# wenet-e2e/wetts

Hardware: AMD Instinct MI355X
Metric: audio samples/sec + RTF @22.05 kHz, VITS-Baker, 1/2/4/8 MI355X (higher is better)
Workload: dtype f32

## Files before the change

wetts_amd/csrc/kernels.h:

```cpp
#pragma once
#include "common.h"

namespace wetts {

int32_t k_embed_mask(const int64_t* ids, const int64_t* lengths, const float* emb, int n_vocab,
                     int B, int H, int T, float* x_out, float* mask_out, int32_t* status,
                     hipStream_t s);

int32_t k_layernorm(const float* a, const float* add, const float* gamma, const float* beta,
                    const float* res, const float* mask, int gelu, int B, int C, int T, float* out,
                    hipStream_t s);

struct DdsFusedParams {
  const float* x;
  float* out;
  const float* mask;
  const float *sep_w[3], *sep_b[3], *n1g[3], *n1b[3], *n2g[3], *n2b[3];
  const float* wpk[3];
  const float* bias[3];
  int B, C, T, G;
};
bool dds_fused_supported(int mode, int C, int Cw, int nchunks, int B, int T);
int32_t k_dds_fused(DdsFusedParams p, hipStream_t s);
int32_t k_dwconv(const float* x, const float* mask, const float* w, const float* bias, int k,
                 int dil, int B, int C, int T, float* out, hipStream_t s, int Tvalid = 0);

int32_t k_cond_linear(const float* g, const float* W, const float* bias, int B, int Cout, int K,
                      float* out, hipStream_t s);

int32_t k_gather_rows(const int64_t* idx, const float* table, int n_rows, int B, int C, float* out,
                      int32_t* status, hipStream_t s);

int32_t k_add_bias_b(float* x, const float* v, int B, int C, int T, hipStream_t s);
int32_t k_add_bias_b_mask(float* x, const float* v, const float* mask, int B, int C, int T,
                          hipStream_t s);
int32_t k_scale(const float* a, float scale, int64_t n, float* out, hipStream_t s);

int32_t k_convflow_pre(const float* z, int ch0, const float* w, const float* bias, const float* g,
                       int B, int C, int T, float* out, hipStream_t s);

int32_t k_spline_inverse(float* z, int ch0, int ch1, const float* h, const float* mask,
                         int num_bins, float tail_bound, float inv_sqrt_div, int B, int T,
                         int32_t* status, hipStream_t s);

int32_t k_affine_reverse(const float* z, int ch, const float* m, const float* logs, int param_idx,
                         const float* mask, int B, int T, float* logw, hipStream_t s);

int32_t k_gate(const float* a, int B, int H, int T, float* out, hipStream_t s);

int32_t k_wn_update(const float* rs, float* h, float* skip, const float* mask, int last, int first,
                    int B, int H, int T, hipStream_t s);

int32_t k_coupling_flip(const float* xin, const float* m, const float* mask, int B, int C, int T,
                        float* out, hipStream_t s);

int32_t k_conv_post_tanh(const float* x, const float* w, int k, int B, int C, int T, float* out,
                         hipStream_t s, const int64_t* lens = nullptr, int len_mul = 0);

int32_t k_durations_to_lengths(const float* logw, const float* mask, float length_scale, int B,
                               int T, float* w_ceil, float* cum, int64_t* y_lengths,
                               int32_t* status, hipStream_t s);

int32_t k_frame_index(const float* cum, const int64_t* y_lengths, int B, int Tx, int Ty,
                      int32_t* frame2phone, float* y_mask, hipStream_t s);
int32_t k_expand_prior(const float* stats, const int32_t* frame2phone, const float* eps,
                       int64_t eps_bs, int64_t eps_cs, float noise_scale, int B, int C, int Tx, int Ty, float* m_exp,
                       float* logs_exp, float* z_p, hipStream_t s);
int32_t k_attn_path(const int32_t* frame2phone, int B, int Tx, int Ty, float* attn, hipStream_t s);

int32_t k_audio_to_int16(const float* audio, const int64_t* lengths, int B, int64_t L, int16_t* pcm,
                         hipStream_t s);

int32_t k_vocos_pad(const float* z, int64_t z_bs, int64_t z_cs, const float* mask,
                    int64_t mask_stride, int B, int C, int L, float* out, hipStream_t s, int Fs = 0);
int32_t k_vocos_spec(const float* spec, int B, int half, int F, float* ri, hipStream_t s, int64_t ri_bs = 0);
int32_t k_istft_basis(int n_fft, float* w, hipStream_t s, double inv_scale = 0.0);
bool k_convnext_dwln(const float* x, const float* w, const float* wb, const float* gamma, const float* beta, int B, int C,
                     int T, int Tvalid, float* out, hipStream_t s, int32_t* rc);
int32_t k_istft_ola(const float* frames, int B, int n_fft, int hop, int F, float* audio,
                    hipStream_t s, int Fs = 0, int envelope = 1);
int32_t k_scale_rows(const float* a, const float* scale, int rows, int cols, float* out,
                     hipStream_t s);

int32_t k_flip_half(const float* x, const float* mask, int B, int C, int T, float* x0, float* x0m,
                    hipStream_t s);
int32_t k_mono_split(const float* x, const float* mask, int B, int C, int T, float sc, float* x0, float* x0m,
                     hipStream_t s);
int32_t k_mono_coupling(const float* x, const float* m, const float* mask, int B, int C, int T, float sc, float* out,
                        hipStream_t s);
int32_t k_coupling_fwd_flip(const float* x, const float* m, const float* mask, int B, int C, int T, float* out,
// ... 35 lines not shown
```

wetts_amd/csrc/kernels.hip:

```cpp
#include "kernels.h"

namespace wetts {

static inline dim3 grid1d(int64_t n, int threads) {
  return dim3((unsigned)((n + threads - 1) / threads));
}

__global__ void embed_mask_kernel(const int64_t* __restrict__ ids,
                                  const int64_t* __restrict__ lengths,
                                  const float* __restrict__ emb, int n_vocab, int B, int H, int T,
                                  float scale, float* __restrict__ x_out,
                                  float* __restrict__ mask_out, int32_t* __restrict__ status) {
  int64_t idx = (int64_t)blockIdx.x * blockDim.x + threadIdx.x;
  int64_t total = (int64_t)B * H * T;
  if (idx >= total) return;
  int t = (int)(idx % T);
  int c = (int)((idx / T) % H);
  int b = (int)(idx / ((int64_t)T * H));
  bool valid = (int64_t)t < lengths[b];
  float v = 0.f;
  if (valid) {
    int64_t id = ids[(int64_t)b * T + t];
    if (id < 0 || id >= n_vocab) {
      if (status && c == 0) atomicOr(status, WETTS_STATUS_PHONE_ID_RANGE);
// ... 663 lines not shown
  const float* xb = x + (int64_t)b * C * T;
  float win[MAXC][K], wv[MAXC][K];
#pragma unroll
  for (int j = 0; j < MAXC; ++j) {
    const int c = cg + CG * j;
    const int cc = c < C ? c : 0;
#pragma unroll
    for (int i = 0; i < K; ++i) {
      const int tt = t - pad + i;
      const bool ok = c < C && tt >= 0 && tt < T;
      win[j][i] = xb[(int64_t)cc * T + (ok ? tt : 0)];
      wv[j][i] = ok ? w[cc * K + i] : 0.f;
    }
  }
  float acc = 0.f;
#pragma unroll
  for (int j = 0; j < MAXC; ++j)
#pragma unroll
    for (int i = 0; i < K; ++i) {
      const float v = win[j][i];
      acc += wv[j][i] * (v > 0.f ? v : v * 0.01f);
    }
  red[cg][tl] = acc;
  __syncthreads();
  if (cg == 0 && t < T) {
    float tot = 0.f;
#pragma unroll
    for (int q = 0; q < CG; ++q) tot += red[q][tl];
    out[(int64_t)b * T + t] = tanhf(tot);
  }
}

int32_t k_conv_post_tanh(const float* x, const float* w, int k, int B, int C, int T, float* out,
                         hipStream_t s, const int64_t* lens, int len_mul) {
  WETTS_REQUIRE(k <= 15, "conv_post kernel size %d unsupported", k);
  int64_t n = (int64_t)B * ((T + 3) / 4);
  if (n == 0) return WETTS_OK;
  if (k == 7 && C <= 64 && n <= 64 * 256 && !lens) {
    hipLaunchKernelGGL(conv_post_tanh_small_kernel<7>, dim3((unsigned)(B * cdiv(T, 32))), dim3(256), 0, s, x, w,
                       B, C, T, out);
    WETTS_LAUNCH_CHECK();
    return WETTS_OK;
  }
  hipLaunchKernelGGL(conv_post_tanh_kernel, grid1d(n, 256), dim3(256), (size_t)C * k * 4, s, x, w,
                     k, B, C, T, out, lens, len_mul);
  WETTS_LAUNCH_CHECK();
  return WETTS_OK;
}

__global__ __launch_bounds__(64) void durations_kernel(const float* __restrict__ logw,
                                                       const float* __restrict__ mask,
                                                       float length_scale, int B, int T,
                                                       float* __restrict__ w_ceil,
                                                       float* __restrict__ cum,
                                                       int64_t* __restrict__ y_lengths,
                                                       int32_t* __restrict__ status) {
  const int b = blockIdx.x, lane = threadIdx.x;
  float carry = 0.f;
  for (int t0 = 0; t0 < T; t0 += 64) {
    int t = t0 + lane;
    float wc = 0.f;
    if (t < T) {
      float w = expf(logw[(int64_t)b * T + t]) * mask[(int64_t)b * T + t] * length_scale;
      wc = ceilf(w);
      w_ceil[(int64_t)b * T + t] = wc;
    }
    float v = wc;
#pragma unroll
    for (int off = 1; off < 64; off <<= 1) {
      float n = __shfl_up(v, off, 64);
      if (lane >= off) v += n;
// ... 548 lines not shown
```

wetts_amd/csrc/model.hip:

```cpp
#include <stdarg.h>
#include <stdlib.h>
#include <string.h>

#include <map>
#include <string>
#include <vector>

#include "common.h"
#include "conv_bf16.h"
#include "resblock32.h"
#include "qconv_u8.h"
#include "kernels.h"

namespace wetts {

static thread_local char g_err[512] = "";

void set_error(const char* fmt, ...) {
  va_list ap;
  va_start(ap, fmt);
  vsnprintf(g_err, sizeof(g_err), fmt, ap);
  va_end(ap);
}

// ... 394 lines not shown
  int fuse32_maxc = 32;
  int fuse32_kmax = 99;
  int fuse32_kwide = 3;
  int fuse2_maxc = 128;
  int fuse_min_blocks = 128;
  int small_max_tiles = 256;
  int chain_whole_waste_pct = 15;
  int chain_whole_maxc = 64;
  int chain_pair_maxc = 32;
  int chain_pair_kmax = 3;
  int fuse2_waste_pct = 20;
  mutable int flow_precision = 0;
  mutable std::vector<std::vector<PackedConvB>> b_wn_in, b_wn_rs;
  mutable PackedConvB b_post;
  mutable float* b_post_wpad = nullptr;
  mutable PackedQConv q_pre, q_cond, q_post;
  mutable std::vector<std::vector<PackedQConv>> q_c1, q_c2;
  mutable bool q_packed = false;
  mutable int flow_packed_prec = 0, dec_packed_prec = 0;
  mutable std::vector<PackedConvB> b_ups;
  mutable PackedConvB b_pre;
  mutable std::vector<std::vector<PackedConvB>> b_c1, b_c2;
  mutable int32_t* status_word = nullptr;
  mutable uint64_t rng_seed = 0, rng_offset = 0;
  int mrf_streams = 1;
  int mrf_fork_maxc = 1 << 20;
  int stage2_pct = 30;
  int dds_fused = 1;
  int wn_gate = 1;
  int wn_fuse = 1;
  int small_fork = 1;
  int conv_groups = 1;
  hipStream_t aux_stream[WETTS_MAX_RB_KERNELS] = {};
  hipEvent_t ev_fork = nullptr, ev_chain[WETTS_MAX_RB_KERNELS] = {};
  bool fork_ok = false;

  int spec_channels = 0;
  bool post_loaded = false;
  Layout post_layout;
  float* post_blob = nullptr;
  PackedConv pe_pre, pe_proj;
  std::vector<PackedConv> pe_in, pe_rs, fwd_pre;
  const float *pe_cond_w = nullptr, *pe_cond_b = nullptr;

  const float* T(const std::string& name) const {
    auto it = layout.index.find(name);
    if (it == layout.index.end()) return nullptr;
    return blob + layout.specs[it->second].offset;
  }
};

namespace wetts {

struct Bump {
  char* base;
  int64_t cap, off = 0;
  bool ok = true;
  Bump(void* p, int64_t c) : base((char*)p), cap(c) {}
  template <typename T>
  T* take(int64_t n) {
    int64_t bytes = align_up(n * (int64_t)sizeof(T), 256);
    if (off + bytes > cap) {
      ok = false;
      return nullptr;
    }
    T* r = (T*)(base + off);
    off += bytes;
    return r;
// ... 426 lines not shown
  return L.total;
}

int32_t wetts_create(const wetts_config_t* cfg, const float* blob_dev, int64_t blob_numel,
                     void* stream, wetts_model_t** out) {
  WETTS_TRY(validate_config(cfg));
  WETTS_REQUIRE(out != nullptr && blob_dev != nullptr, "null argument");
  hipStream_t s = (hipStream_t)stream;
  wetts_model* m = new wetts_model();
  m->cfg = *cfg;
  build_layout(cfg, m->layout);
  if (blob_numel != m->layout.total) {
    set_error("blob has %lld floats, layout needs %lld", (long long)blob_numel,
              (long long)m->layout.total);
    delete m;
    return WETTS_E_INVALID;
  }
  hipError_t e = hipMalloc((void**)&m->blob, (size_t)blob_numel * sizeof(float));
  if (e != hipSuccess) {
    set_error("hipMalloc(blob) failed: %s", hipGetErrorString(e));
    delete m;
    return WETTS_E_HIP;
  }
  e = hipMemcpyAsync(m->blob, blob_dev, (size_t)blob_numel * sizeof(float),
                     hipMemcpyDeviceToDevice, s);
  int32_t r = (e == hipSuccess) ? build_model(m, s) : WETTS_E_HIP;
  {
    struct Knob { const char* name; int* field; };
    const Knob knobs[] = {
        {"stage2_pct", &m->stage2_pct}, {"dds_fused", &m->dds_fused}, {"wn_fuse", &m->wn_fuse}, {"wn_gate", &m->wn_gate},
        {"fuse2_waste_pct", &m->fuse2_waste_pct}, {"fuse_min_blocks", &m->fuse_min_blocks},
        {"chain_whole_pct", &m->chain_whole_waste_pct}, {"chain_whole_maxc", &m->chain_whole_maxc},
        {"small_max_tiles", &m->small_max_tiles},
    };
    if (const char* env = getenv("WETTS_TUNE")) {
      std::string all(env);
      size_t pos = 0;
      while (pos < all.size()) {
        size_t end = all.find(',', pos);
        if (end == std::string::npos) end = all.size();
        const std::string item = all.substr(pos, end - pos);
        const size_t eq = item.find('=');
        bool known = false;
        if (eq != std::string::npos)
          for (const Knob& k : knobs)
            if (item.compare(0, eq, k.name) == 0 && strlen(k.name) == eq) {
              *k.field = atoi(item.c_str() + eq + 1);
              known = true;
            }
        if (!known && !item.empty()) {
          set_error("WETTS_TUNE: unknown setting '%s'", item.c_str());
          r = WETTS_E_INVALID;
        }
        pos = end + 1;
      }
    }
    if (r == WETTS_OK && !m->wn_gate) {
      const int H = cfg->hidden_channels, fk = cfg->flow_kernel_size;
      for (int f = 0; f < cfg->flow_n_flows && r == WETTS_OK; ++f)
        for (int i = 0; i < cfg->flow_wn_layers && r == WETTS_OK; ++i) {
          const std::string p = S("flow.flows.%d.enc.in_layers.%d", flow_key_stride(cfg) * f, i);
          free_packed(&m->flows[f].in_layers[i]);
          r = pack_conv_weight(m->T(p + ".weight"), m->T(p + ".bias"), 2 * H, H, fk, 1, (fk - 1) / 2, 0, 0, s,
                               &m->flows[f].in_layers[i]);
        }
    }
    if (m->mrf_streams < 1) m->mrf_streams = 1;
    if (m->mrf_streams > cfg->n_resblock_kernels) m->mrf_streams = cfg->n_resblock_kernels;
    m->fork_ok = hipEventCreateWithFlags(&m->ev_fork, hipEventDisableTiming) == hipSuccess && m->ev_fork;
    for (int j = 0; j < cfg->n_resblock_kernels; ++j) {
      if (hipEventCreateWithFlags(&m->ev_chain[j], hipEventDisableTiming) != hipSuccess || !m->ev_chain[j]) m->fork_ok = false;
      if (j > 0)
        if (hipStreamCreateWithFlags(&m->aux_stream[j], hipStreamNonBlocking) != hipSuccess || !m->aux_stream[j]) m->fork_ok = false;
    }
    (void)hipGetLastError();
  }
  if (r == WETTS_OK) {
    e = hipStreamSynchronize(s);
    if (e != hipSuccess) {
      set_error("weight packing failed: %s", hipGetErrorString(e));
      r = WETTS_E_HIP;
    }
  }
  if (r != WETTS_OK) {
    wetts_destroy(m);
    return r;
  }
  *out = m;
  return WETTS_OK;
}

void wetts_destroy(wetts_model_t* m) {
  if (!m) return;
  free_posterior(m);
  for (PackedConv* pc : m->all_packed) free_packed(pc);
  for (auto& pc : m->b_ups) free_packed_bf16(&pc);
  for (auto& v : m->b_c1) for (auto& pc : v) free_packed_bf16(&pc);
  for (auto& v : m->b_c2) for (auto& pc : v) free_packed_bf16(&pc);
  for (auto& v : m->b_wn_in) for (auto& pc : v) free_packed_bf16(&pc);
  for (auto& v : m->b_wn_rs) for (auto& pc : v) free_packed_bf16(&pc);
  free_packed_bf16(&m->b_post);
  if (m->b_post_wpad) (void)hipFree(m->b_post_wpad);
  free_packed_qconv(&m->q_pre);
  free_packed_qconv(&m->q_cond);
  free_packed_qconv(&m->q_post);
  for (auto& v : m->q_c1) for (auto& pc : v) free_packed_qconv(&pc);
  for (auto& v : m->q_c2) for (auto& pc : v) free_packed_qconv(&pc);
  for (int j = 0; j < WETTS_MAX_RB_KERNELS; ++j) {
    if (m->aux_stream[j]) (void)hipStreamDestroy(m->aux_stream[j]);
    if (m->ev_chain[j]) (void)hipEventDestroy(m->ev_chain[j]);
  }
  if (m->ev_fork) (void)hipEventDestroy(m->ev_fork);
  for (float* p : m->v_owned) (void)hipFree(p);
  if (m->blob) (void)hipFree(m->blob);
  delete m;
}

int32_t wetts_hop_length(const wetts_model_t* m) { return m ? m->hop : WETTS_E_INVALID; }

int32_t wetts_set_istft_mode(const wetts_model_t* m, int32_t mode) {
  WETTS_REQUIRE(m, "null model");
  WETTS_REQUIRE(mode == WETTS_ISTFT_TORCH || mode == WETTS_ISTFT_ONNX, "istft mode must be 0 (torch.istft) or 1 (OnnxSTFT.inverse), got %d", mode);
  m->istft_mode = mode;
  return WETTS_OK;
}

int32_t wetts_get_istft_mode(const wetts_model_t* m) { return m ? m->istft_mode : WETTS_E_INVALID; }

int32_t wetts_get_blob(const wetts_model_t* m, float* out_dev, int64_t numel, void* stream) {
  WETTS_REQUIRE(m && out_dev, "null argument");
  WETTS_REQUIRE(numel == m->layout.total, "blob has %lld floats, asked for %lld", (long long)m->layout.total,
                (long long)numel);
  WETTS_HIP_CHECK(hipMemcpyAsync(out_dev, m->blob, (size_t)numel * sizeof(float), hipMemcpyDeviceToDevice,
                                 (hipStream_t)stream));
  return WETTS_OK;
}

int64_t wetts_workspace_bytes(const wetts_model_t* m, int32_t B, int32_t Tx, int32_t Ty) {
  if (!m || B < 0 || Tx < 0 || Ty < 0) return WETTS_E_INVALID;
  const wetts_config_t* c = &m->cfg;
  int64_t a = ws_encoder(c, B, Tx);
  int64_t b = c->use_sdp ? ws_sdp(c, B, Tx) : ws_dp(c, B, Tx);
  int64_t need = a > b ? a : b;
  if (Ty > 0) {
    int64_t f = ws_flow(c, B, Ty), d = ws_decoder(c, B, Ty);
// ... 1001 lines not shown
        WETTS_TRY(launch_resblock_pair32(rb.c1[d], rb.c2[d], pp, s));
        count(1, 2 + accum);
      } else {
        ConvParams p2 = conv_io(chain_buf[j][2], ch, len, outp[j], ch, B);
        p2.in_act = IN_LRELU;
        p2.in_slope = 0.1f;
        p2.res = rx[j];
        p2.r_bs = (int64_t)ch * len;
        p2.r_cs = len;
        p2.accum = accum;
        p2.out_div = odiv;
        p2.tag = 1;
        p2.lens = lens;
        p2.len_mul = spf;
        if (last_d || m->dec_unfused) {
          WETTS_TRY(launch_conv(rb.c2[d], p2, s));
          count(1, 3 + accum);
        } else {
          g2[n2] = &rb.c2[d];
          p2s[n2++] = p2;
        }
      }
      rx[j] = outp[j];
    }
    if (n2 > 0) {
      int nl = 0;
      WETTS_TRY(launch_conv_group(g2, p2s, n2, s, &nl));
      count(nl, 3.0 * n2);
    }
  }
  return WETTS_OK;
}

static int32_t run_hifigan(const wetts_model* m, const float* z, int64_t z_bs, int64_t z_cs,
                           const float* y_mask, int64_t mask_stride, const float* g, int B, int L,
                           float* audio, void* workspace, int64_t workspace_bytes, hipStream_t s,
                           DecTiming* tm, const int64_t* lens = nullptr) {
  const wetts_config_t* c = &m->cfg;
  const int I = c->inter_channels, C0 = c->upsample_initial_channel;
  const int64_t mx = dec_max_elems(c, B, L);
  Bump ws(workspace, workspace_bytes);
  float* bx = ws.take<float>(mx);
  float* bt = ws.take<float>(mx);
  float* bs = ws.take<float>(mx);
  float* chain_buf[WETTS_MAX_RB_KERNELS][3];
  for (int j = 0; j < c->n_resblock_kernels; ++j)
    for (int q = 0; q < 3; ++q) chain_buf[j][q] = ws.take<float>(mx);
  float* cond = ws.take<float>((int64_t)B * C0);
  if (!ws.ok) {
    set_error("hifigan: workspace too small (need %lld bytes)",
              (long long)ws_decoder(c, B, L));
    return WETTS_E_WORKSPACE;
  }
  {
    ConvParams p = conv_io(z, I, L, bx, C0, B);
    p.x_bs = z_bs;
    p.x_cs = z_cs;
    if (y_mask) {
      p.in_mask = y_mask;
      p.in_mask_stride = mask_stride;
    }
    if (has_g(c) && g) {
      WETTS_TRY(k_cond_linear(g, m->dec_cond_w, m->dec_cond_b, B, C0, c->gin_channels, cond, s));
      p.bias_b = cond;
      p.bias_b_stride = C0;
    }
    p.lens = lens;
    p.len_mul = 1;
    WETTS_TRY(launch_conv(m->conv_pre, p, s));
  }
  int ch = C0, len = L;
  int spf = 1;
  float* x = bx;
  float* xs = bs;
  const int nk = c->n_resblock_kernels, nd = c->n_resblock_dilations;
  for (int i = 0; i < c->n_upsamples; ++i) {
    const int u = c->upsample_rates[i];
    {
      ConvParams p = conv_io(x, ch, len, bt, ch / 2, B);
      p.in_act = IN_LRELU;
      p.in_slope = 0.1f;
      p.Tout = len * u;
      p.o_bs = (int64_t)(ch / 2) * len * u;
      p.o_cs = (int64_t)len * u;
      p.lens = lens;
      p.len_mul = spf;
      WETTS_TRY(launch_conv(m->ups[i], p, s));
    }
    ch /= 2;
    len *= u;
    spf *= u;
    float* xu = bt;
    float* xsum = (x == bx) ? bs : bx;
    (void)xs;
    if (tm && tm->on) WETTS_HIP_CHECK(hipEventRecord(tm->e0, s));
    hipEvent_t lv0 = nullptr, lv1 = nullptr;
    if (m->mrf_timing) {
      WETTS_HIP_CHECK(hipEventCreate(&lv0));
      WETTS_HIP_CHECK(hipEventCreate(&lv1));
      WETTS_HIP_CHECK(hipEventRecord(lv0, s));
    }
    const bool small_stage = !lens && (int64_t)cdiv(ch, 64) * cdiv(len, 64) * B <= m->small_max_tiles;
    const int nstreams = !m->fork_ok ? 1 : (c->resblock == 1 && ((m->small_fork && small_stage) || (ch <= m->mrf_fork_maxc && !m->dec_serial))) ? nk : m->mrf_streams;
    const bool forked = nstreams > 1;
    if (forked) WETTS_HIP_CHECK(hipEventRecord(m->ev_fork, s));
    const bool chain_addr_ok = (int64_t)ch * len * 4 < (int64_t)INT32_MAX;
    const bool grouped = c->resblock == 1 && !forked && m->conv_groups;
    if (grouped) WETTS_TRY(run_stage_rb1_grouped(m, i, xu, xsum, chain_buf, ch, len, spf, B, lens, tm, s));
    for (int j = 0; j < (grouped ? 0 : nk); ++j) {
      const RB& rb = m->rbs[i * nk + j];
      hipStream_t sj = (forked && j > 0 && j < nstreams) ? m->aux_stream[j] : s;
      if (sj != s) WETTS_HIP_CHECK(hipStreamWaitEvent(sj, m->ev_fork, 0));
      float* fa = chain_buf[j][0];
      float* fb = chain_buf[j][1];
      float* ft = chain_buf[j][2];
      const float* rx = xu;
      if (c->resblock == 1 && !m->dec_unfused && nd <= RESCHAIN32_MAX_PAIRS &&
          ch <= m->chain_whole_maxc && m->chain_whole_waste_pct > 0 && len % 4 == 0 && chain_addr_ok &&
          resblock_chain32_supported(rb.c1.data(), rb.c2.data(), nd, m->fuse32_lds / 2,
                                     m->chain_whole_waste_pct)) {
        int dl[RESCHAIN32_MAX_PAIRS];
        for (int d = 0; d < nd; ++d) dl[d] = rb.c1[d].dil;
        if (cdiv(len, resblock_chain32_nto(ch, rb.c1[0].ktaps, dl, nd)) * B >= m->fuse_min_blocks) {
          ResChain32Params cp;
          memset(&cp, 0, sizeof(cp));
          cp.x = rx;
          cp.out = xsum;
          cp.T = len;
          cp.B = B;
          cp.accum = (j > 0) ? 1 : 0;
          cp.out_div = (j == nk - 1) ? (float)nk : 1.f;
          cp.slope = 0.1f;
          cp.lens = lens;
          cp.len_mul = spf;
          if (forked && j > 0) WETTS_HIP_CHECK(hipStreamWaitEvent(sj, m->ev_chain[j - 1], 0));
          WETTS_TRY(launch_resblock_chain32(rb.c1.data(), rb.c2.data(), nd, cp, sj));
          if (forked) WETTS_HIP_CHECK(hipEventRecord(m->ev_chain[j], sj));
          if (tm && tm->on) tm->launches += 1;
          mrf_count(m, 1, 2 + (j > 0 ? 1 : 0), ch, len, B, 4);
          continue;
        }
      }
      for (int d = 0; d < nd; ++d) {
        const bool last_d = (d == nd - 1);
        float* outp;
        int accum = 0;
        float odiv = 1.f;
        if (last_d) {
          outp = xsum;
          accum = (j > 0) ? 1 : 0;
          odiv = (j == nk - 1) ? (float)nk : 1.f;
        } else {
          outp = (rx == fa) ? fb : fa;
        }
        if (c->resblock == 2 && nd == 2 && d == 0 && !m->dec_unfused && !forked &&
            ch <= m->fuse2_maxc &&
            resblock2_chain32_supported(rb.c1[0], rb.c1[1], m->fuse32_lds,
                                        ch <= 32 ? m->fuse2_waste_pct : (m->fuse2_waste_pct + 1) / 2) &&
            cdiv(len, pair_nto(ch, 1) - (rb.c1[1].ktaps - 1) * rb.c1[1].dil) * B >= m->fuse_min_blocks) {
          ResPair32Params pp;
          memset(&pp, 0, sizeof(pp));
          pp.x = rx;
          pp.out = xsum;
          pp.T = len;
          pp.B = B;
          pp.accum = (j > 0) ? 1 : 0;
          pp.out_div = (j == nk - 1) ? (float)nk : 1.f;
          pp.slope = 0.1f;
          WETTS_TRY(launch_resblock2_chain32(rb.c1[0], rb.c1[1], pp, sj));
          if (tm && tm->on) tm->launches += 1;
          mrf_count(m, 1, 2 + (j > 0 ? 1 : 0), ch, len, B, 4);
          rx = xsum;
          break;
        }
        const int pair_tiles = cdiv(len, pair_nto(ch, rb.c1[d].ktaps)) * B;
        const bool chain1 = c->resblock == 1 && !m->dec_unfused && len % 4 == 0 && chain_addr_ok &&
                            (ch <= m->chain_pair_maxc || rb.c1[d].ktaps <= m->chain_pair_kmax) &&
                            resblock_chain32_supported(&rb.c1[d], &rb.c2[d], 1, m->fuse32_lds / 2, 100) &&
                            pair_tiles >= m->fuse_min_blocks;
        if (chain1) {
          if (forked && last_d && j > 0) WETTS_HIP_CHECK(hipStreamWaitEvent(sj, m->ev_chain[j - 1], 0));
          ResChain32Params cp;
          memset(&cp, 0, sizeof(cp));
          cp.x = rx;
          cp.out = outp;
          cp.T = len;
          cp.B = B;
          cp.accum = accum;
          cp.out_div = odiv;
          cp.slope = 0.1f;
          cp.lens = lens;
          cp.len_mul = spf;
          WETTS_TRY(launch_resblock_chain32(&rb.c1[d], &rb.c2[d], 1, cp, sj));
          if (tm && tm->on) tm->launches += 1;
          mrf_count(m, 1, 2 + accum, ch, len, B, 4);
          rx = outp;
          continue;
        }
        const bool fuse32 = c->resblock == 1 && !m->dec_unfused && !lens &&
                            resblock_pair32_supported(rb.c1[d], rb.c2[d], m->fuse32_lds) &&
                            !(ch >= 128 && rb.c1[d].ktaps >= m->fuse32_kmax128) &&
                            (ch <= m->fuse32_maxc || rb.c1[d].ktaps <= m->fuse32_kwide) &&
                            rb.c1[d].ktaps <= m->fuse32_kmax &&
                            pair_tiles >= m->fuse_min_blocks;
        if (fuse32) {
          if (forked && last_d && j > 0) WETTS_HIP_CHECK(hipStreamWaitEvent(sj, m->ev_chain[j - 1], 0));
          ResPair32Params pp;
          memset(&pp, 0, sizeof(pp));
          pp.x = rx;
          pp.out = outp;
          pp.T = len;
          pp.B = B;
          pp.accum = accum;
          pp.out_div = odiv;
          pp.slope = 0.1f;
          WETTS_TRY(launch_resblock_pair32(rb.c1[d], rb.c2[d], pp, sj));
          if (tm && tm->on) tm->launches += 1;
          mrf_count(m, 1, 2 + accum, ch, len, B, 4);
        } else if (c->resblock == 1) {
          ConvParams p1 = conv_io(rx, ch, len, ft, ch, B);
          p1.in_act = IN_LRELU;
          p1.in_slope = 0.1f;
          p1.tag = 1;
          p1.lens = lens;
          p1.len_mul = spf;
          WETTS_TRY(launch_conv(rb.c1[d], p1, sj));
          if (forked && last_d && j > 0) WETTS_HIP_CHECK(hipStreamWaitEvent(sj, m->ev_chain[j - 1], 0));
          ConvParams p2 = conv_io(ft, ch, len, outp, ch, B);
          p2.in_act = IN_LRELU;
          p2.in_slope = 0.1f;
          p2.res = rx;
          p2.r_bs = (int64_t)ch * len;
          p2.r_cs = len;
          p2.accum = accum;
          p2.out_div = odiv;
          p2.tag = 1;
          p2.lens = lens;
          p2.len_mul = spf;
          WETTS_TRY(launch_conv(rb.c2[d], p2, sj));
          if (tm && tm->on) tm->launches += 2;
          mrf_count(m, 2, 5 + accum, ch, len, B, 4);
        } else {
          if (forked && last_d && j > 0) WETTS_HIP_CHECK(hipStreamWaitEvent(sj, m->ev_chain[j - 1], 0));
          ConvParams p1 = conv_io(rx, ch, len, outp, ch, B);
          p1.in_act = IN_LRELU;
          p1.in_slope = 0.1f;
          p1.res = rx;
          p1.r_bs = (int64_t)ch * len;
          p1.r_cs = len;
          p1.accum = accum;
          p1.out_div = odiv;
          p1.tag = 1;
          WETTS_TRY(launch_conv(rb.c1[d], p1, sj));
          if (tm && tm->on) tm->launches += 1;
          mrf_count(m, 1, 2 + accum, ch, len, B, 4);
        }
        rx = outp;
      }
      if (forked) WETTS_HIP_CHECK(hipEventRecord(m->ev_chain[j], sj));
    }
    if (forked) WETTS_HIP_CHECK(hipStreamWaitEvent(s, m->ev_chain[nk - 1], 0));
    if (m->mrf_timing) {
      WETTS_HIP_CHECK(hipEventRecord(lv1, s));
      m->mrf_events.emplace_back(lv0, lv1);
    }
    if (tm && tm->on) {
      WETTS_HIP_CHECK(hipEventRecord(tm->e1, s));
      WETTS_HIP_CHECK(hipEventSynchronize(tm->e1));
      float ms = 0.f;
      WETTS_HIP_CHECK(hipEventElapsedTime(&ms, tm->e0, tm->e1));
      tm->mrf_ms += ms;
    }
    x = xsum;
  }
  WETTS_TRY(k_conv_post_tanh(x, m->conv_post_w, 7, B, ch, len, audio, s, lens, spf));
  if (m->mrf_timing) m->mrf_calls += 1;
  return WETTS_OK;
}
}

namespace wetts {
static void free_decoder_bf16(const wetts_model* m) {
  for (auto& pc : m->b_ups) free_packed_bf16(&pc);
  for (auto& v : m->b_c1) for (auto& pc : v) free_packed_bf16(&pc);
  for (auto& v : m->b_c2) for (auto& pc : v) free_packed_bf16(&pc);
  free_packed_bf16(&m->b_post);
  free_packed_bf16(&m->b_pre);
  m->b_ups.clear();
  m->b_c1.clear();
  m->b_c2.clear();
  m->dec_packed_prec = 0;
}

static int32_t pack_decoder_bf16_layers(const wetts_model* m, int f16, hipStream_t s) {
  const wetts_config_t* c = &m->cfg;
  const int nk = c->n_resblock_kernels, nd = c->n_resblock_dilations;
  m->b_ups.resize(c->n_upsamples);
  m->b_c1.assign(c->n_upsamples * nk, std::vector<PackedConvB>(nd));
  m->b_c2.assign(c->n_upsamples * nk, std::vector<PackedConvB>(c->resblock == 1 ? nd : 0));
  int ch = c->upsample_initial_channel;
  WETTS_TRY(pack_conv_weight_bf16(m->T("dec.conv_pre.weight"), m->T("dec.conv_pre.bias"), ch, c->inter_channels, 7, 1, 3,
                                  0, 0, f16, s, &m->b_pre));
  for (int i = 0; i < c->n_upsamples; ++i) {
    const int u = c->upsample_rates[i], uk = c->upsample_kernel_sizes[i];
    WETTS_TRY(pack_conv_weight_bf16(m->T(S("dec.ups.%d.weight", i)), m->T(S("dec.ups.%d.bias", i)),
                                    ch / 2, ch, uk, 1, (uk - u) / 2, 1, u, f16, s, &m->b_ups[i]));
    ch /= 2;
    for (int j = 0; j < nk; ++j) {
// ... 784 lines not shown
```

Before: 52.71 million.

## Split HiFi-GAN decoder batch into two slices run concurrently on separate streams

Refactors the decoder into per-slice stage helpers (conv_pre, upsample, resblock chains, join, conv_post) and adds a path that splits the batch into two halves whose stages are issued interleaved with separate fork/chain events. Each half can then overlap the other's kernels on separate streams, filling the GPU when a single batch's kernels leave it underused. It is gated by a tunable dec_split and skipped when the per-half stages would be too small. The cost is extra event and stream synchronisation, smaller kernels per launch, and more complex buffer handling per slice.

```diff
diff --git a/wetts_amd/csrc/kernels.h b/wetts_amd/csrc/kernels.h
--- a/wetts_amd/csrc/kernels.h
+++ b/wetts_amd/csrc/kernels.h
@@ -55,7 +55,7 @@
                         float* out, hipStream_t s);
 
 int32_t k_conv_post_tanh(const float* x, const float* w, int k, int B, int C, int T, float* out,
-                         hipStream_t s, const int64_t* lens = nullptr, int len_mul = 0);
+                         hipStream_t s, const int64_t* lens = nullptr, int len_mul = 0, int sel_rows = 0);
 
 int32_t k_durations_to_lengths(const float* logw, const float* mask, float length_scale, int B,
                                int T, float* w_ceil, float* cum, int64_t* y_lengths,
diff --git a/wetts_amd/csrc/kernels.hip b/wetts_amd/csrc/kernels.hip
--- a/wetts_amd/csrc/kernels.hip
+++ b/wetts_amd/csrc/kernels.hip
@@ -719,11 +719,12 @@
 }
 
 int32_t k_conv_post_tanh(const float* x, const float* w, int k, int B, int C, int T, float* out,
-                         hipStream_t s, const int64_t* lens, int len_mul) {
+                         hipStream_t s, const int64_t* lens, int len_mul, int sel_rows) {
   WETTS_REQUIRE(k <= 15, "conv_post kernel size %d unsupported", k);
   int64_t n = (int64_t)B * ((T + 3) / 4);
   if (n == 0) return WETTS_OK;
-  if (k == 7 && C <= 64 && n <= 64 * 256 && !lens) {
+  const int64_t n_sel = (int64_t)(sel_rows > 0 ? sel_rows : B) * ((T + 3) / 4);
+  if (k == 7 && C <= 64 && n_sel <= 64 * 256 && !lens) {
     hipLaunchKernelGGL(conv_post_tanh_small_kernel<7>, dim3((unsigned)(B * cdiv(T, 32))), dim3(256), 0, s, x, w,
                        B, C, T, out);
     WETTS_LAUNCH_CHECK();
diff --git a/wetts_amd/csrc/model.hip b/wetts_amd/csrc/model.hip
--- a/wetts_amd/csrc/model.hip
+++ b/wetts_amd/csrc/model.hip
@@ -450,8 +450,10 @@
   int small_fork = 1;
   int conv_groups = 1;
   hipStream_t aux_stream[WETTS_MAX_RB_KERNELS] = {};
-  hipEvent_t ev_fork = nullptr, ev_chain[WETTS_MAX_RB_KERNELS] = {};
+  hipEvent_t ev_fork[2] = {}, ev_chain[2][WETTS_MAX_RB_KERNELS] = {};
   bool fork_ok = false;
+  int dec_split = 1;
+  int dec_split_min_rows = 2;
 
   int spec_channels = 0;
   bool post_loaded = false;
@@ -944,6 +946,7 @@
         {"fuse2_waste_pct", &m->fuse2_waste_pct}, {"fuse_min_blocks", &m->fuse_min_blocks},
         {"chain_whole_pct", &m->chain_whole_waste_pct}, {"chain_whole_maxc", &m->chain_whole_maxc},
         {"small_max_tiles", &m->small_max_tiles},
+        {"dec_split", &m->dec_split}, {"dec_split_min_rows", &m->dec_split_min_rows},
     };
     if (const char* env = getenv("WETTS_TUNE")) {
       std::string all(env);
@@ -979,9 +982,13 @@
     }
     if (m->mrf_streams < 1) m->mrf_streams = 1;
     if (m->mrf_streams > cfg->n_resblock_kernels) m->mrf_streams = cfg->n_resblock_kernels;
-    m->fork_ok = hipEventCreateWithFlags(&m->ev_fork, hipEventDisableTiming) == hipSuccess && m->ev_fork;
+    m->fork_ok = true;
+    for (int h = 0; h < 2; ++h) {
+      if (hipEventCreateWithFlags(&m->ev_fork[h], hipEventDisableTiming) != hipSuccess || !m->ev_fork[h]) m->fork_ok = false;
+      for (int j = 0; j < cfg->n_resblock_kernels; ++j)
+        if (hipEventCreateWithFlags(&m->ev_chain[h][j], hipEventDisableTiming) != hipSuccess || !m->ev_chain[h][j]) m->fork_ok = false;
+    }
     for (int j = 0; j < cfg->n_resblock_kernels; ++j) {
-      if (hipEventCreateWithFlags(&m->ev_chain[j], hipEventDisableTiming) != hipSuccess || !m->ev_chain[j]) m->fork_ok = false;
       if (j > 0)
         if (hipStreamCreateWithFlags(&m->aux_stream[j], hipStreamNonBlocking) != hipSuccess || !m->aux_stream[j]) m->fork_ok = false;
     }
@@ -1020,9 +1027,11 @@
   for (auto& v : m->q_c2) for (auto& pc : v) free_packed_qconv(&pc);
   for (int j = 0; j < WETTS_MAX_RB_KERNELS; ++j) {
     if (m->aux_stream[j]) (void)hipStreamDestroy(m->aux_stream[j]);
-    if (m->ev_chain[j]) (void)hipEventDestroy(m->ev_chain[j]);
-  }
-  if (m->ev_fork) (void)hipEventDestroy(m->ev_fork);
+    for (int h = 0; h < 2; ++h)
+      if (m->ev_chain[h][j]) (void)hipEventDestroy(m->ev_chain[h][j]);
+  }
+  for (int h = 0; h < 2; ++h)
+    if (m->ev_fork[h]) (void)hipEventDestroy(m->ev_fork[h]);
   for (float* p : m->v_owned) (void)hipFree(p);
   if (m->blob) (void)hipFree(m->blob);
   delete m;
@@ -2090,19 +2099,283 @@
   return WETTS_OK;
 }
 
+struct DecSlice {
+  int B = 0;
+  int Bsel = 0;
+  const float* z = nullptr;
+  const float* y_mask = nullptr;
+  const float* cond = nullptr;
+  const int64_t* lens = nullptr;
+  float* audio = nullptr;
+  float *bx = nullptr, *bt = nullptr, *bs = nullptr;
+  float* chain_buf[WETTS_MAX_RB_KERNELS][3] = {};
+  hipEvent_t ev_fork = nullptr;
+  const hipEvent_t* ev_chain = nullptr;
+  int ch = 0, len = 0, spf = 1;
+  float* x = nullptr;
+  float* xsum = nullptr;
+  bool forked = false;
+};
+
+static int32_t dec_conv_pre(const wetts_model* m, DecSlice& sl, int64_t z_bs, int64_t z_cs, int64_t mask_stride, int L,
+                            hipStream_t s) {
+  const wetts_config_t* c = &m->cfg;
+  const int C0 = c->upsample_initial_channel;
+  ConvParams p = conv_io(sl.z, c->inter_channels, L, sl.bx, C0, sl.B);
+  p.x_bs = z_bs;
+  p.x_cs = z_cs;
+  if (sl.y_mask) {
+    p.in_mask = sl.y_mask;
+    p.in_mask_stride = mask_stride;
+  }
+  if (sl.cond) {
+    p.bias_b = sl.cond;
+    p.bias_b_stride = C0;
+  }
+  p.lens = sl.lens;
+  p.len_mul = 1;
+  WETTS_TRY(launch_conv(m->conv_pre, p, s));
+  sl.ch = C0;
+  sl.len = L;
+  sl.spf = 1;
+  sl.x = sl.bx;
+  return WETTS_OK;
+}
+
+static int32_t dec_upsample(const wetts_model* m, DecSlice& sl, int i, hipStream_t s) {
+  const int u = m->cfg.upsample_rates[i];
+  const int ch = sl.ch, len = sl.len;
+  ConvParams p = conv_io(sl.x, ch, len, sl.bt, ch / 2, sl.B);
+  p.in_act = IN_LRELU;
+  p.in_slope = 0.1f;
+  p.Tout = len * u;
+  p.o_bs = (int64_t)(ch / 2) * len * u;
+  p.o_cs = (int64_t)len * u;
+  p.lens = sl.lens;
+  p.len_mul = sl.spf;
+  WETTS_TRY(launch_conv(m->ups[i], p, s));
+  sl.ch = ch / 2;
+  sl.len = len * u;
+  sl.spf *= u;
+  return WETTS_OK;
+}
+
+static int32_t dec_stage_chains(const wetts_model* m, DecSlice& sl, int i, DecTiming* tm, hipStream_t s) {
+  const wetts_config_t* c = &m->cfg;
+  const int nk = c->n_resblock_kernels, nd = c->n_resblock_dilations;
+  const int ch = sl.ch, len = sl.len, spf = sl.spf, B = sl.B, Bsel = sl.Bsel;
+  const int64_t* lens = sl.lens;
+  float* xu = sl.bt;
+  float* xsum = (sl.x == sl.bx) ? sl.bs : sl.bx;
+  sl.xsum = xsum;
+  const bool small_stage = !lens && (int64_t)cdiv(ch, 64) * cdiv(len, 64) * Bsel <= m->small_max_tiles;
+  const int nstreams = !m->fork_ok ? 1 : (c->resblock == 1 && ((m->small_fork && small_stage) || (ch <= m->mrf_fork_maxc && !m->dec_serial))) ? nk : m->mrf_streams;
+  const bool forked = nstreams > 1;
+  sl.forked = forked;
+  if (forked) WETTS_HIP_CHECK(hipEventRecord(sl.ev_fork, s));
+  const bool chain_addr_ok = (int64_t)ch * len * 4 < (int64_t)INT32_MAX;
+  const bool grouped = c->resblock == 1 && !forked && m->conv_groups;
+  if (grouped) WETTS_TRY(run_stage_rb1_grouped(m, i, xu, xsum, sl.chain_buf, ch, len, spf, B, lens, tm, s));
+  for (int j = 0; j < (grouped ? 0 : nk); ++j) {
+    const RB& rb = m->rbs[i * nk + j];
+    hipStream_t sj = (forked && j > 0 && j < nstreams) ? m->aux_stream[j] : s;
+    if (sj != s) WETTS_HIP_CHECK(hipStreamWaitEvent(sj, sl.ev_fork, 0));
+    float* fa = sl.chain_buf[j][0];
+    float* fb = sl.chain_buf[j][1];
+    float* ft = sl.chain_buf[j][2];
+    const float* rx = xu;
+    if (c->resblock == 1 && !m->dec_unfused && nd <= RESCHAIN32_MAX_PAIRS &&
+        ch <= m->chain_whole_maxc && m->chain_whole_waste_pct > 0 && len % 4 == 0 && chain_addr_ok &&
+        resblock_chain32_supported(rb.c1.data(), rb.c2.data(), nd, m->fuse32_lds / 2,
+                                   m->chain_whole_waste_pct)) {
+      int dl[RESCHAIN32_MAX_PAIRS];
+      for (int d = 0; d < nd; ++d) dl[d] = rb.c1[d].dil;
+      if (cdiv(len, resblock_chain32_nto(ch, rb.c1[0].ktaps, dl, nd)) * Bsel >= m->fuse_min_blocks) {
+        ResChain32Params cp;
+        memset(&cp, 0, sizeof(cp));
+        cp.x = rx;
+        cp.out = xsum;
+        cp.T = len;
+        cp.B = B;
+        cp.accum = (j > 0) ? 1 : 0;
+        cp.out_div = (j == nk - 1) ? (float)nk : 1.f;
+        cp.slope = 0.1f;
+        cp.lens = lens;
+        cp.len_mul = spf;
+        if (forked && j > 0) WETTS_HIP_CHECK(hipStreamWaitEvent(sj, sl.ev_chain[j - 1], 0));
+        WETTS_TRY(launch_resblock_chain32(rb.c1.data(), rb.c2.data(), nd, cp, sj));
+        if (forked) WETTS_HIP_CHECK(hipEventRecord(sl.ev_chain[j], sj));
+        if (tm && tm->on) tm->launches += 1;
+        mrf_count(m, 1, 2 + (j > 0 ? 1 : 0), ch, len, B, 4);
+        continue;
+      }
+    }
+    for (int d = 0; d < nd; ++d) {
+      const bool last_d = (d == nd - 1);
+      float* outp;
+      int accum = 0;
+      float odiv = 1.f;
+      if (last_d) {
+        outp = xsum;
+        accum = (j > 0) ? 1 : 0;
+        odiv = (j == nk - 1) ? (float)nk : 1.f;
+      } else {
+        outp = (rx == fa) ? fb : fa;
+      }
+      if (c->resblock == 2 && nd == 2 && d == 0 && !m->dec_unfused && !forked &&
+          ch <= m->fuse2_maxc &&
+          resblock2_chain32_supported(rb.c1[0], rb.c1[1], m->fuse32_lds,
+                                      ch <= 32 ? m->fuse2_waste_pct : (m->fuse2_waste_pct + 1) / 2) &&
+          cdiv(len, pair_nto(ch, 1) - (rb.c1[1].ktaps - 1) * rb.c1[1].dil) * Bsel >= m->fuse_min_blocks) {
+        ResPair32Params pp;
+        memset(&pp, 0, sizeof(pp));
+        pp.x = rx;
+        pp.out = xsum;
+        pp.T = len;
+        pp.B = B;
+        pp.accum = (j > 0) ? 1 : 0;
+        pp.out_div = (j == nk - 1) ? (float)nk : 1.f;
+        pp.slope = 0.1f;
+        WETTS_TRY(launch_resblock2_chain32(rb.c1[0], rb.c1[1], pp, sj));
+        if (tm && tm->on) tm->launches += 1;
+        mrf_count(m, 1, 2 + (j > 0 ? 1 : 0), ch, len, B, 4);
+        rx = xsum;
+        break;
+      }
+      const int pair_tiles = cdiv(len, pair_nto(ch, rb.c1[d].ktaps)) * Bsel;
+      const bool chain1 = c->resblock == 1 && !m->dec_unfused && len % 4 == 0 && chain_addr_ok &&
+                          (ch <= m->chain_pair_maxc || rb.c1[d].ktaps <= m->chain_pair_kmax) &&
+                          resblock_chain32_supported(&rb.c1[d], &rb.c2[d], 1, m->fuse32_lds / 2, 100) &&
+                          pair_tiles >= m->fuse_min_blocks;
+      if (chain1) {
+        if (forked && last_d && j > 0) WETTS_HIP_CHECK(hipStreamWaitEvent(sj, sl.ev_chain[j - 1], 0));
+        ResChain32Params cp;
+        memset(&cp, 0, sizeof(cp));
+        cp.x = rx;
+        cp.out = outp;
+        cp.T = len;
+        cp.B = B;
+        cp.accum = accum;
+        cp.out_div = odiv;
+        cp.slope = 0.1f;
+        cp.lens = lens;
+        cp.len_mul = spf;
+        WETTS_TRY(launch_resblock_chain32(&rb.c1[d], &rb.c2[d], 1, cp, sj));
+        if (tm && tm->on) tm->launches += 1;
+        mrf_count(m, 1, 2 + accum, ch, len, B, 4);
+        rx = outp;
+        continue;
+      }
+      const bool fuse32 = c->resblock == 1 && !m->dec_unfused && !lens &&
+                          resblock_pair32_supported(rb.c1[d], rb.c2[d], m->fuse32_lds) &&
+                          !(ch >= 128 && rb.c1[d].ktaps >= m->fuse32_kmax128) &&
+                          (ch <= m->fuse32_maxc || rb.c1[d].ktaps <= m->fuse32_kwide) &&
+                          rb.c1[d].ktaps <= m->fuse32_kmax &&
+                          pair_tiles >= m->fuse_min_blocks;
+      if (fuse32) {
+        if (forked && last_d && j > 0) WETTS_HIP_CHECK(hipStreamWaitEvent(sj, sl.ev_chain[j - 1], 0));
+        ResPair32Params pp;
+        memset(&pp, 0, sizeof(pp));
+        pp.x = rx;
+        pp.out = outp;
+        pp.T = len;
+        pp.B = B;
+        pp.accum = accum;
+        pp.out_div = odiv;
+        pp.slope = 0.1f;
+        WETTS_TRY(launch_resblock_pair32(rb.c1[d], rb.c2[d], pp, sj));
+        if (tm && tm->on) tm->launches += 1;
+        mrf_count(m, 1, 2 + accum, ch, len, B, 4);
+      } else if (c->resblock == 1) {
+        ConvParams p1 = conv_io(rx, ch, len, ft, ch, B);
+        p1.in_act = IN_LRELU;
+        p1.in_slope = 0.1f;
+        p1.tag = 1;
+        p1.lens = lens;
+        p1.len_mul = spf;
+        WETTS_TRY(launch_conv(rb.c1[d], p1, sj));
+        if (forked && last_d && j > 0) WETTS_HIP_CHECK(hipStreamWaitEvent(sj, sl.ev_chain[j - 1], 0));
+        ConvParams p2 = conv_io(ft, ch, len, outp, ch, B);
+        p2.in_act = IN_LRELU;
+        p2.in_slope = 0.1f;
+        p2.res = rx;
+        p2.r_bs = (int64_t)ch * len;
+        p2.r_cs = len;
+        p2.accum = accum;
+        p2.out_div = odiv;
+        p2.tag = 1;
+        p2.lens = lens;
+        p2.len_mul = spf;
+        WETTS_TRY(launch_conv(rb.c2[d], p2, sj));
+        if (tm && tm->on) tm->launches += 2;
+        mrf_count(m, 2, 5 + accum, ch, len, B, 4);
+      } else {
+        if (forked && last_d && j > 0) WETTS_HIP_CHECK(hipStreamWaitEvent(sj, sl.ev_chain[j - 1], 0));
+        ConvParams p1 = conv_io(rx, ch, len, outp, ch, B);
+        p1.in_act = IN_LRELU;
+        p1.in_slope = 0.1f;
+        p1.res = rx;
+        p1.r_bs = (int64_t)ch * len;
+        p1.r_cs = len;
+        p1.accum = accum;
+        p1.out_div = odiv;
+        p1.tag = 1;
+        WETTS_TRY(launch_conv(rb.c1[d], p1, sj));
+        if (tm && tm->on) tm->launches += 1;
+        mrf_count(m, 1, 2 + accum, ch, len, B, 4);
+      }
+      rx = outp;
+    }
+    if (forked) WETTS_HIP_CHECK(hipEventRecord(sl.ev_chain[j], sj));
+  }
+  return WETTS_OK;
+}
+
+static int32_t dec_stage_join(const wetts_model* m, DecSlice& sl, hipStream_t s) {
+  if (sl.forked) WETTS_HIP_CHECK(hipStreamWaitEvent(s, sl.ev_chain[m->cfg.n_resblock_kernels - 1], 0));
+  sl.x = sl.xsum;
+  return WETTS_OK;
+}
+
+static int32_t dec_conv_post(const wetts_model* m, DecSlice& sl, hipStream_t s) {
+  return k_conv_post_tanh(sl.x, m->conv_post_w, 7, sl.B, sl.ch, sl.len, sl.audio, s, sl.lens, sl.spf, sl.Bsel);
+}
+
+static int dec_split_rows(const wetts_model* m, int B, int L, bool ragged, const DecTiming* tm) {
+  const wetts_config_t* c = &m->cfg;
+  if (!m->dec_split || !m->fork_ok || m->dec_serial || m->dec_unfused || (tm && tm->on)) return 0;
+  if (B < 2 || B < m->dec_split_min_rows) return 0;
+  if (c->resblock != 1 || c->n_upsamples < 1 || c->upsample_initial_channel > m->mrf_fork_maxc) return 0;
+  if ((dec_max_elems(c, B, L) / B) % 4 != 0) return 0;
+  if (!ragged) {
+    const int64_t Bs = B / 2, smt = m->small_max_tiles;
+    int64_t ch = c->upsample_initial_channel, len = L;
+    if (cdiv((int)ch, 64) * (int64_t)cdiv((int)len, 64) * Bs <= smt) return 0;
+    for (int i = 0; i < c->n_upsamples; ++i) {
+      const int u = c->upsample_rates[i];
+      if (cdiv((int)(ch / 2 * u), 64) * (int64_t)cdiv((int)len, 64) * Bs <= smt) return 0;
+      ch /= 2;
+      len *= u;
+      if (cdiv((int)ch, 64) * (int64_t)cdiv((int)len, 64) * Bs <= smt) return 0;
+    }
+  }
+  return (B + 1) / 2;
+}
+
 static int32_t run_hifigan(const wetts_model* m, const float* z, int64_t z_bs, int64_t z_cs,
                            const float* y_mask, int64_t mask_stride, const float* g, int B, int L,
                            float* audio, void* workspace, int64_t workspace_bytes, hipStream_t s,
                            DecTiming* tm, const int64_t* lens = nullptr) {
   const wetts_config_t* c = &m->cfg;
-  const int I = c->inter_channels, C0 = c->upsample_initial_channel;
+  const int C0 = c->upsample_initial_channel;
+  const int nk = c->n_resblock_kernels, nup = c->n_upsamples;
   const int64_t mx = dec_max_elems(c, B, L);
   Bump ws(workspace, workspace_bytes);
   float* bx = ws.take<float>(mx);
   float* bt = ws.take<float>(mx);
   float* bs = ws.take<float>(mx);
   float* chain_buf[WETTS_MAX_RB_KERNELS][3];
-  for (int j = 0; j < c->n_resblock_kernels; ++j)
+  for (int j = 0; j < nk; ++j)
     for (int q = 0; q < 3; ++q) chain_buf[j][q] = ws.take<float>(mx);
   float* cond = ws.take<float>((int64_t)B * C0);
   if (!ws.ok) {
@@ -2110,47 +2383,67 @@
               (long long)ws_decoder(c, B, L));
     return WETTS_E_WORKSPACE;
   }
-  {
-    ConvParams p = conv_io(z, I, L, bx, C0, B);
-    p.x_bs = z_bs;
-    p.x_cs = z_cs;
-    if (y_mask) {
-      p.in_mask = y_mask;
-      p.in_mask_stride = mask_stride;
-    }
-    if (has_g(c) && g) {
-      WETTS_TRY(k_cond_linear(g, m->dec_cond_w, m->dec_cond_b, B, C0, c->gin_channels, cond, s));
-      p.bias_b = cond;
-      p.bias_b_stride = C0;
-    }
-    p.lens = lens;
-    p.len_mul = 1;
-    WETTS_TRY(launch_conv(m->conv_pre, p, s));
-  }
-  int ch = C0, len = L;
-  int spf = 1;
-  float* x = bx;
-  float* xs = bs;
-  const int nk = c->n_resblock_kernels, nd = c->n_resblock_dilations;
-  for (int i = 0; i < c->n_upsamples; ++i) {
-    const int u = c->upsample_rates[i];
-    {
-      ConvParams p = conv_io(x, ch, len, bt, ch / 2, B);
-      p.in_act = IN_LRELU;
-      p.in_slope = 0.1f;
-      p.Tout = len * u;
-      p.o_bs = (int64_t)(ch / 2) * len * u;
-      p.o_cs = (int64_t)len * u;
-      p.lens = lens;
-      p.len_mul = spf;
-      WETTS_TRY(launch_conv(m->ups[i], p, s));
-    }
-    ch /= 2;
-    len *= u;
-    spf *= u;
-    float* xu = bt;
-    float* xsum = (x == bx) ? bs : bx;
-    (void)xs;
+  const bool has_cond = has_g(c) && g;
+  if (has_cond) WETTS_TRY(k_cond_linear(g, m->dec_cond_w, m->dec_cond_b, B, C0, c->gin_channels, cond, s));
+  int64_t audio_len = L;
+  for (int i = 0; i < nup; ++i) audio_len *= c->upsample_rates[i];
+  auto make_slice = [&](int h, int r0, int rows) {
+    DecSlice sl;
+    const int64_t base = (int64_t)r0 * (mx / B);
+    sl.B = rows;
+    sl.Bsel = B;
+    sl.z = z + (int64_t)r0 * z_bs;
+    sl.y_mask = y_mask ? y_mask + (int64_t)r0 * mask_stride : nullptr;
+    sl.cond = has_cond ? cond + (int64_t)r0 * C0 : nullptr;
+    sl.lens = lens ? lens + r0 : nullptr;
+    sl.audio = audio + (int64_t)r0 * audio_len;
+    sl.bx = bx + base;
+    sl.bt = bt + base;
+    sl.bs = bs + base;
+    for (int j = 0; j < nk; ++j)
+      for (int q = 0; q < 3; ++q) sl.chain_buf[j][q] = chain_buf[j][q] + base;
+    sl.ev_fork = m->ev_fork[h];
+    sl.ev_chain = m->ev_chain[h];
+    return sl;
+  };
+  const int rows_a = dec_split_rows(m, B, L, lens != nullptr, tm);
+  if (rows_a > 0) {
+    DecSlice sa = make_slice(0, 0, rows_a), sb = make_slice(1, rows_a, B - rows_a);
+    hipEvent_t lv0 = nullptr, lv1 = nullptr;
+    WETTS_TRY(dec_conv_pre(m, sa, z_bs, z_cs, mask_stride, L, s));
+    WETTS_TRY(dec_upsample(m, sa, 0, s));
+    if (m->mrf_timing) {
+      WETTS_HIP_CHECK(hipEventCreate(&lv0));
+      WETTS_HIP_CHECK(hipEventCreate(&lv1));
+      WETTS_HIP_CHECK(hipEventRecord(lv0, s));
+    }
+    WETTS_TRY(dec_stage_chains(m, sa, 0, tm, s));
+    WETTS_TRY(dec_conv_pre(m, sb, z_bs, z_cs, mask_stride, L, s));
+    WETTS_TRY(dec_upsample(m, sb, 0, s));
+    WETTS_TRY(dec_stage_chains(m, sb, 0, tm, s));
+    for (int i = 1; i < nup; ++i) {
+      WETTS_TRY(dec_stage_join(m, sa, s));
+      WETTS_TRY(dec_upsample(m, sa, i, s));
+      WETTS_TRY(dec_stage_chains(m, sa, i, tm, s));
+      WETTS_TRY(dec_stage_join(m, sb, s));
+      WETTS_TRY(dec_upsample(m, sb, i, s));
+      WETTS_TRY(dec_stage_chains(m, sb, i, tm, s));
+    }
+    WETTS_TRY(dec_stage_join(m, sa, s));
+    WETTS_TRY(dec_conv_post(m, sa, s));
+    WETTS_TRY(dec_stage_join(m, sb, s));
+    if (m->mrf_timing) {
+      WETTS_HIP_CHECK(hipEventRecord(lv1, s));
+      m->mrf_events.emplace_back(lv0, lv1);
+    }
+    WETTS_TRY(dec_conv_post(m, sb, s));
+    if (m->mrf_timing) m->mrf_calls += 1;
+    return WETTS_OK;
+  }
+  DecSlice sl = make_slice(0, 0, B);
+  WETTS_TRY(dec_conv_pre(m, sl, z_bs, z_cs, mask_stride, L, s));
+  for (int i = 0; i < nup; ++i) {
+    WETTS_TRY(dec_upsample(m, sl, i, s));
     if (tm && tm->on) WETTS_HIP_CHECK(hipEventRecord(tm->e0, s));
     hipEvent_t lv0 = nullptr, lv1 = nullptr;
     if (m->mrf_timing) {
@@ -2158,166 +2451,8 @@
       WETTS_HIP_CHECK(hipEventCreate(&lv1));
       WETTS_HIP_CHECK(hipEventRecord(lv0, s));
     }
-    const bool small_stage = !lens && (int64_t)cdiv(ch, 64) * cdiv(len, 64) * B <= m->small_max_tiles;
-    const int nstreams = !m->fork_ok ? 1 : (c->resblock == 1 && ((m->small_fork && small_stage) || (ch <= m->mrf_fork_maxc && !m->dec_serial))) ? nk : m->mrf_streams;
-    const bool forked = nstreams > 1;
-    if (forked) WETTS_HIP_CHECK(hipEventRecord(m->ev_fork, s));
-    const bool chain_addr_ok = (int64_t)ch * len * 4 < (int64_t)INT32_MAX;
-    const bool grouped = c->resblock == 1 && !forked && m->conv_groups;
-    if (grouped) WETTS_TRY(run_stage_rb1_grouped(m, i, xu, xsum, chain_buf, ch, len, spf, B, lens, tm, s));
-    for (int j = 0; j < (grouped ? 0 : nk); ++j) {
-      const RB& rb = m->rbs[i * nk + j];
-      hipStream_t sj = (forked && j > 0 && j < nstreams) ? m->aux_stream[j] : s;
-      if (sj != s) WETTS_HIP_CHECK(hipStreamWaitEvent(sj, m->ev_fork, 0));
-      float* fa = chain_buf[j][0];
-      float* fb = chain_buf[j][1];
-      float* ft = chain_buf[j][2];
-      const float* rx = xu;
-      if (c->resblock == 1 && !m->dec_unfused && nd <= RESCHAIN32_MAX_PAIRS &&
-          ch <= m->chain_whole_maxc && m->chain_whole_waste_pct > 0 && len % 4 == 0 && chain_addr_ok &&
-          resblock_chain32_supported(rb.c1.data(), rb.c2.data(), nd, m->fuse32_lds / 2,
-                                     m->chain_whole_waste_pct)) {
-        int dl[RESCHAIN32_MAX_PAIRS];
-        for (int d = 0; d < nd; ++d) dl[d] = rb.c1[d].dil;
-        if (cdiv(len, resblock_chain32_nto(ch, rb.c1[0].ktaps, dl, nd)) * B >= m->fuse_min_blocks) {
-          ResChain32Params cp;
-          memset(&cp, 0, sizeof(cp));
-          cp.x = rx;
-          cp.out = xsum;
-          cp.T = len;
-          cp.B = B;
-          cp.accum = (j > 0) ? 1 : 0;
-          cp.out_div = (j == nk - 1) ? (float)nk : 1.f;
-          cp.slope = 0.1f;
-          cp.lens = lens;
-          cp.len_mul = spf;
-          if (forked && j > 0) WETTS_HIP_CHECK(hipStreamWaitEvent(sj, m->ev_chain[j - 1], 0));
-          WETTS_TRY(launch_resblock_chain32(rb.c1.data(), rb.c2.data(), nd, cp, sj));
-          if (forked) WETTS_HIP_CHECK(hipEventRecord(m->ev_chain[j], sj));
-          if (tm && tm->on) tm->launches += 1;
-          mrf_count(m, 1, 2 + (j > 0 ? 1 : 0), ch, len, B, 4);
-          continue;
-        }
-      }
-      for (int d = 0; d < nd; ++d) {
-        const bool last_d = (d == nd - 1);
-        float* outp;
-        int accum = 0;
-        float odiv = 1.f;
-        if (last_d) {
-          outp = xsum;
-          accum = (j > 0) ? 1 : 0;
-          odiv = (j == nk - 1) ? (float)nk : 1.f;
-        } else {
-          outp = (rx == fa) ? fb : fa;
-        }
-        if (c->resblock == 2 && nd == 2 && d == 0 && !m->dec_unfused && !forked &&
-            ch <= m->fuse2_maxc &&
-            resblock2_chain32_supported(rb.c1[0], rb.c1[1], m->fuse32_lds,
-                                        ch <= 32 ? m->fuse2_waste_pct : (m->fuse2_waste_pct + 1) / 2) &&
-            cdiv(len, pair_nto(ch, 1) - (rb.c1[1].ktaps - 1) * rb.c1[1].dil) * B >= m->fuse_min_blocks) {
-          ResPair32Params pp;
-          memset(&pp, 0, sizeof(pp));
-          pp.x = rx;
-          pp.out = xsum;
-          pp.T = len;
-          pp.B = B;
-          pp.accum = (j > 0) ? 1 : 0;
-          pp.out_div = (j == nk - 1) ? (float)nk : 1.f;
-          pp.slope = 0.1f;
-          WETTS_TRY(launch_resblock2_chain32(rb.c1[0], rb.c1[1], pp, sj));
-          if (tm && tm->on) tm->launches += 1;
-          mrf_count(m, 1, 2 + (j > 0 ? 1 : 0), ch, len, B, 4);
-          rx = xsum;
-          break;
-        }
-        const int pair_tiles = cdiv(len, pair_nto(ch, rb.c1[d].ktaps)) * B;
-        const bool chain1 = c->resblock == 1 && !m->dec_unfused && len % 4 == 0 && chain_addr_ok &&
-                            (ch <= m->chain_pair_maxc || rb.c1[d].ktaps <= m->chain_pair_kmax) &&
-                            resblock_chain32_supported(&rb.c1[d], &rb.c2[d], 1, m->fuse32_lds / 2, 100) &&
-                            pair_tiles >= m->fuse_min_blocks;
-        if (chain1) {
-          if (forked && last_d && j > 0) WETTS_HIP_CHECK(hipStreamWaitEvent(sj, m->ev_chain[j - 1], 0));
-          ResChain32Params cp;
-          memset(&cp, 0, sizeof(cp));
-          cp.x = rx;
-          cp.out = outp;
-          cp.T = len;
-          cp.B = B;
-          cp.accum = accum;
-          cp.out_div = odiv;
-          cp.slope = 0.1f;
-          cp.lens = lens;
-          cp.len_mul = spf;
-          WETTS_TRY(launch_resblock_chain32(&rb.c1[d], &rb.c2[d], 1, cp, sj));
-          if (tm && tm->on) tm->launches += 1;
-          mrf_count(m, 1, 2 + accum, ch, len, B, 4);
-          rx = outp;
-          continue;
-        }
-        const bool fuse32 = c->resblock == 1 && !m->dec_unfused && !lens &&
-                            resblock_pair32_supported(rb.c1[d], rb.c2[d], m->fuse32_lds) &&
-                            !(ch >= 128 && rb.c1[d].ktaps >= m->fuse32_kmax128) &&
-                            (ch <= m->fuse32_maxc || rb.c1[d].ktaps <= m->fuse32_kwide) &&
-                            rb.c1[d].ktaps <= m->fuse32_kmax &&
-                            pair_tiles >= m->fuse_min_blocks;
-        if (fuse32) {
-          if (forked && last_d && j > 0) WETTS_HIP_CHECK(hipStreamWaitEvent(sj, m->ev_chain[j - 1], 0));
-          ResPair32Params pp;
-          memset(&pp, 0, sizeof(pp));
-          pp.x = rx;
-          pp.out = outp;
-          pp.T = len;
-          pp.B = B;
-          pp.accum = accum;
-          pp.out_div = odiv;
-          pp.slope = 0.1f;
-          WETTS_TRY(launch_resblock_pair32(rb.c1[d], rb.c2[d], pp, sj));
-          if (tm && tm->on) tm->launches += 1;
-          mrf_count(m, 1, 2 + accum, ch, len, B, 4);
-        } else if (c->resblock == 1) {
-          ConvParams p1 = conv_io(rx, ch, len, ft, ch, B);
-          p1.in_act = IN_LRELU;
-          p1.in_slope = 0.1f;
-          p1.tag = 1;
-          p1.lens = lens;
-          p1.len_mul = spf;
-          WETTS_TRY(launch_conv(rb.c1[d], p1, sj));
-          if (forked && last_d && j > 0) WETTS_HIP_CHECK(hipStreamWaitEvent(sj, m->ev_chain[j - 1], 0));
-          ConvParams p2 = conv_io(ft, ch, len, outp, ch, B);
-          p2.in_act = IN_LRELU;
-          p2.in_slope = 0.1f;
-          p2.res = rx;
-          p2.r_bs = (int64_t)ch * len;
-          p2.r_cs = len;
-          p2.accum = accum;
-          p2.out_div = odiv;
-          p2.tag = 1;
-          p2.lens = lens;
-          p2.len_mul = spf;
-          WETTS_TRY(launch_conv(rb.c2[d], p2, sj));
-          if (tm && tm->on) tm->launches += 2;
-          mrf_count(m, 2, 5 + accum, ch, len, B, 4);
-        } else {
-          if (forked && last_d && j > 0) WETTS_HIP_CHECK(hipStreamWaitEvent(sj, m->ev_chain[j - 1], 0));
-          ConvParams p1 = conv_io(rx, ch, len, outp, ch, B);
-          p1.in_act = IN_LRELU;
-          p1.in_slope = 0.1f;
-          p1.res = rx;
-          p1.r_bs = (int64_t)ch * len;
-          p1.r_cs = len;
-          p1.accum = accum;
-          p1.out_div = odiv;
-          p1.tag = 1;
-          WETTS_TRY(launch_conv(rb.c1[d], p1, sj));
-          if (tm && tm->on) tm->launches += 1;
-          mrf_count(m, 1, 2 + accum, ch, len, B, 4);
-        }
-        rx = outp;
-      }
-      if (forked) WETTS_HIP_CHECK(hipEventRecord(m->ev_chain[j], sj));
-    }
-    if (forked) WETTS_HIP_CHECK(hipStreamWaitEvent(s, m->ev_chain[nk - 1], 0));
+    WETTS_TRY(dec_stage_chains(m, sl, i, tm, s));
+    WETTS_TRY(dec_stage_join(m, sl, s));
     if (m->mrf_timing) {
       WETTS_HIP_CHECK(hipEventRecord(lv1, s));
       m->mrf_events.emplace_back(lv0, lv1);
@@ -2329,9 +2464,8 @@
       WETTS_HIP_CHECK(hipEventElapsedTime(&ms, tm->e0, tm->e1));
       tm->mrf_ms += ms;
     }
-    x = xsum;
-  }
-  WETTS_TRY(k_conv_post_tanh(x, m->conv_post_w, 7, B, ch, len, audio, s, lens, spf));
+  }
+  WETTS_TRY(dec_conv_post(m, sl, s));
   if (m->mrf_timing) m->mrf_calls += 1;
   return WETTS_OK;
 }
```

New measurement: 51.37 million. -2.5%, worse.
